# HDembinski/zenflow

Hardware: AMD Instinct MI355X
Metric: log_prob samples/sec (+ NLL match) 4D 16-knot 4-layer flow, batch 2^20 (higher is better)
Workload: dtype fp32 (f16x2 split MFMA, fp32 accumulate)

## Files before the change

include/zenflow_amd.h:

```cpp
#ifndef ZENFLOW_AMD_H
#define ZENFLOW_AMD_H

#include <stddef.h>
#include <stdint.h>

#ifdef __cplusplus
extern "C" {
#endif

#define ZF_OK 0
#define ZF_EINVAL (-1)
#define ZF_ENOTSUP (-2)
#define ZF_ENOMEM (-3)

const char* zf_last_error(void);
int zf_version(void);
int zf_device_count(int* count);
int zf_set_device(int device);
int zf_get_device(int* device);
int zf_device_name(int device, char* buf, int buflen);
int zf_device_synchronize(void);
int zf_malloc(void** ptr, size_t bytes);
int zf_free(void* ptr);
int zf_memset_async(void* ptr, int value, size_t bytes, void* stream);
// ... 69 lines not shown
  int32_t cond_dim;
  int32_t latent;
  float latent_param;
  int32_t n_ops;
  int32_t _pad;
  zf_op_desc ops[64];
} zf_flow_desc;

typedef struct zf_flow zf_flow_t;

int zf_flow_plan(zf_flow_desc* desc, int64_t* blob_floats);

int zf_flow_create(const zf_flow_desc* desc, const float* blob_host, int64_t blob_floats,
                   zf_flow_t** handle);
int zf_flow_destroy(zf_flow_t* handle);

#define ZF_KERNEL_FP32 0
#define ZF_KERNEL_BF16X3 1
#define ZF_KERNEL_F16X2 2
#define ZF_KERNEL_LAYERED 3
int zf_flow_kernel_variant(const zf_flow_t* h);

int64_t zf_flow_workspace_bytes(int64_t N);

int zf_flow_log_prob(zf_flow_t* h, const float* x, const float* c, float* log_prob,
                     double* nll_sum, void* workspace, int64_t N, void* stream);

int zf_flow_log_prob_segment(zf_flow_t* h, int op_begin, int op_end, const float* x,
                             const float* c, const float* log_det_in, float* log_prob,
                             double* nll_sum, void* workspace, int64_t N, void* stream);

int zf_flow_nll_reduce(const void* workspace, int64_t N, double* nll_sum, void* stream);

int zf_flow_forward(zf_flow_t* h, int op_begin, int op_end, const float* x, const float* c,
                    float* y, const float* log_det_in, float* log_det, int64_t N,
                    void* stream);

int zf_flow_inverse(zf_flow_t* h, int op_begin, int op_end, const float* z, const float* c,
                    float* x, int64_t N, void* stream);

int zf_flow_sample(zf_flow_t* h, uint64_t seed, const float* c, float* x, int64_t N, void* stream);

int zf_latent_sample(int latent, double param, uint64_t seed, float* z, int64_t N, int D, void* stream);

int zf_flow_set_bn_stats(zf_flow_t* h, int op, const float* mean, const float* var);

int zf_flow_set_sb_stats(zf_flow_t* h, int op, const float* xmin, const float* xmax);

int64_t zf_colstats_workspace_bytes(int64_t N, int ncols);
int zf_colstats(const float* x, int64_t N, int ncols, int64_t ld, int col_offset,
                const float* pre_modes, const float* pre_params, float* cmin, float* cmax,
                double* csum, double* csumsq, void* workspace, void* stream);


typedef struct zf_optim_desc {
  float learning_rate, b1, b2, eps, weight_decay;
  int nesterov;
} zf_optim_desc;

typedef struct zf_trainer zf_trainer_t;

int zf_trainer_create(const zf_flow_desc* desc, const float* blob_host, int64_t blob_floats,
                      const unsigned char* param_mask, int64_t batch_max, const zf_optim_desc* opt,
                      zf_trainer_t** trainer);
int zf_trainer_destroy(zf_trainer_t* trainer);

// ... 44 lines not shown
```

zenflow_amd/_lib.py:

```python

from __future__ import annotations

import ctypes as C
import os
import threading
import weakref
from pathlib import Path
from typing import Optional, Sequence, Tuple, Union

import numpy as np

_HERE = Path(__file__).resolve().parent
LIB_PATH = Path(os.environ.get("ZF_LIB", _HERE / "libzenflow_amd.so"))

ZF_OP_SHIFT_BOUNDS = 1
ZF_OP_ROLL = 2
ZF_OP_NSC = 3
ZF_LATENT_NONE = 0
ZF_LATENT_NORMAL = 1
ZF_LATENT_BETA = 2
ZF_LATENT_TRUNCNORM = 3
ZF_LATENT_UNIFORM = 4
ZF_ACT_SWISH = 0
ZF_ACT_RELU = 1
ZF_ACT_TANH = 2
ZF_ACT_SIGMOID = 3
ZF_ACT_GELU = 4
ZF_ACT_SOFTPLUS = 5
ZF_ACT_ELU = 6
ZF_ACT_LEAKY_RELU = 7
ZF_SB_NONE = 0
ZF_SB_BOTH = 1
ZF_SB_LOWER = 2
ZF_SB_UPPER = 3
ZF_KERNEL_FP32 = 0
ZF_KERNEL_BF16X3 = 1
ZF_KERNEL_F16X2 = 2
ZF_KERNEL_LAYERED = 3


class ZfOpDesc(C.Structure):
    _fields_ = [
        ("kind", C.c_int32),
        ("shift", C.c_int32),
        ("knots", C.c_int32),
        ("n_hidden", C.c_int32),
        ("hidden", C.c_int32 * 16),
        ("act", C.c_int32),
        ("_pad", C.c_int32),
        ("off_bn", C.c_int64),
        ("off_w", C.c_int64 * 17),
        ("off_b", C.c_int64 * 17),
        ("off_sb", C.c_int64),
    ]


class ZfOptimDesc(C.Structure):
    _fields_ = [("learning_rate", C.c_float), ("b1", C.c_float), ("b2", C.c_float), ("eps", C.c_float),
                ("weight_decay", C.c_float), ("nesterov", C.c_int)]


ALLGATHER_FN = C.CFUNCTYPE(C.c_int, C.c_void_p, C.c_void_p, C.c_void_p, C.c_size_t, C.c_void_p)


class ZfCommDesc(C.Structure):
    _fields_ = [("rank", C.c_int), ("world", C.c_int), ("ctx", C.c_void_p), ("allgather", C.c_void_p)]


class ZfFlowDesc(C.Structure):
    _fields_ = [
        ("dim", C.c_int32),
# ... 18 lines not shown
    "zf_device_count": (_int, [C.POINTER(_int)]),
    "zf_set_device": (_int, [_int]),
    "zf_get_device": (_int, [C.POINTER(_int)]),
    "zf_device_name": (_int, [_int, C.c_char_p, _int]),
    "zf_device_synchronize": (_int, []),
    "zf_malloc": (_int, [C.POINTER(_vp), C.c_size_t]),
    "zf_free": (_int, [_vp]),
    "zf_memset_async": (_int, [_vp, _int, C.c_size_t, _vp]),
    "zf_memcpy_htod": (_int, [_vp, _vp, C.c_size_t, _vp]),
    "zf_memcpy_dtoh": (_int, [_vp, _vp, C.c_size_t, _vp]),
    "zf_memcpy_dtod": (_int, [_vp, _vp, C.c_size_t, _vp]),
    "zf_stream_create": (_int, [C.POINTER(_vp)]),
    "zf_stream_destroy": (_int, [_vp]),
    "zf_stream_synchronize": (_int, [_vp]),
    "zf_event_create": (_int, [C.POINTER(_vp)]),
    "zf_event_destroy": (_int, [_vp]),
    "zf_event_record": (_int, [_vp, _vp]),
    "zf_stream_wait_event": (_int, [_vp, _vp]),
    "zf_event_elapsed_ms": (_int, [_vp, _vp, C.POINTER(C.c_float)]),
    "zf_event_synchronize": (_int, [_vp]),
    "zf_rqs_forward": (_int, [_vp, _vp, _vp, _vp, _vp, _vp, _i64, _int, _int, _vp]),
    "zf_rqs_inverse": (_int, [_vp, _vp, _vp, _vp, _vp, _i64, _int, _int, _vp]),
    "zf_normalize_spline_params": (_int, [_vp, _vp, _vp, _i64, _int, _vp]),
    "zf_squareplus": (_int, [_vp, _vp, _i64, C.c_float, _vp]),
    "zf_softmax_with_threshold": (_int, [_vp, _vp, _i64, _int, C.c_double, _vp]),
    "zf_flow_plan": (_int, [C.POINTER(ZfFlowDesc), C.POINTER(_i64)]),
    "zf_flow_create": (_int, [C.POINTER(ZfFlowDesc), _vp, _i64, C.POINTER(_vp)]),
    "zf_flow_destroy": (_int, [_vp]),
    "zf_flow_kernel_variant": (_int, [_vp]),
    "zf_flow_workspace_bytes": (_i64, [_i64]),
    "zf_flow_log_prob": (_int, [_vp, _vp, _vp, _vp, _vp, _vp, _i64, _vp]),
    "zf_flow_log_prob_segment": (_int, [_vp, _int, _int, _vp, _vp, _vp, _vp, _vp, _vp, _i64, _vp]),
    "zf_flow_nll_reduce": (_int, [_vp, _i64, _vp, _vp]),
    "zf_flow_forward": (_int, [_vp, _int, _int, _vp, _vp, _vp, _vp, _vp, _i64, _vp]),
    "zf_flow_inverse": (_int, [_vp, _int, _int, _vp, _vp, _vp, _i64, _vp]),
    "zf_flow_sample": (_int, [_vp, _u64, _vp, _vp, _i64, _vp]),
    "zf_trainer_create": (_int, [_vp, _vp, _i64, _vp, _i64, _vp, _vp]),
    "zf_trainer_destroy": (_int, [_vp]),
    "zf_trainer_loss_grad": (_int, [_vp, _vp, _vp, _i64, _int, _vp, _vp, _vp]),
    "zf_trainer_step": (_int, [_vp, _vp, _vp, _i64, _vp, _vp]),
    "zf_trainer_set_comm": (_int, [_vp, _vp]),
    "zf_trainer_loss_grad_shard": (_int, [_vp, _vp, _vp, _i64, _i64, _int, _vp, _vp, _vp]),
    "zf_trainer_step_shard": (_int, [_vp, _vp, _vp, _i64, _i64, _vp, _vp]),
    "zf_trainer_loss_grad_cond_shard": (_int, [_vp, _vp, _vp, _i64, _i64, _int, _vp, _vp, _vp, _vp]),
    "zf_trainer_step_cond_shard": (_int, [_vp, _vp, _vp, _i64, _i64, _vp, _vp, _vp]),
    "zf_trainer_log_prob_vjp": (_int, [_vp, _vp, _vp, _vp, _vp, _vp, _vp, _i64, _vp]),
    "zf_trainer_get_blob": (_int, [_vp, _vp]),
    "zf_trainer_set_blob": (_int, [_vp, _vp]),
    "zf_latent_sample": (_int, [_int, _dbl, _u64, _vp, _i64, _int, _vp]),
    "zf_flow_set_bn_stats": (_int, [_vp, _int, _vp, _vp]),
    "zf_flow_set_sb_stats": (_int, [_vp, _int, _vp, _vp]),
    "zf_colstats_workspace_bytes": (_i64, [_i64, _int]),
    "zf_colstats": (_int, [_vp, _i64, _int, _i64, _int, _vp, _vp, _vp, _vp, _vp, _vp, _vp, _vp]),
    "zf_rccl_available": (_int, []),
    "zf_rccl_get_unique_id": (_int, [C.c_char_p]),
    "zf_rccl_comm_init": (_int, [C.POINTER(_vp), _int, C.c_char_p, _int]),
    "zf_rccl_allreduce_sum_f64": (_int, [_vp, _vp, _vp, C.c_size_t, _vp]),
    "zf_rccl_comm_destroy": (_int, [_vp]),
    "zf_rccl_allgather": (_int, [_vp, _vp, _vp, C.c_size_t, _vp]),
}

_lib: Optional[C.CDLL] = None
_lock = threading.Lock()


def load_library() -> C.CDLL:
# ... 207 lines not shown
```

zenflow_amd/csrc/zf_flow.hip:

```cpp
#include "zf_flow_dev.h"

#include <cmath>
#include <cstdlib>
#include <cstring>
#include <vector>

namespace zf {
namespace {

constexpr int kWaves = 4;
constexpr int kBlockRows = kWaves * kTile;

template <int T>
__device__ __forceinline__ floatx16 mfma_tile(const floatx4* __restrict__ p,
                                              const floatx4* __restrict__ pnext, floatx4 (&cur)[4],
                                              const floatx16 (&hb)[T]) {
  floatx16 acc = floatx16{0};
#pragma unroll
  for (int t = 0; t < T; ++t) {
    floatx4 nxt[4];
    const bool more = (t + 1 < T);
    const floatx4* src = more ? p + (t + 1) * 256 : pnext;
    const bool have = more || (pnext != nullptr);
    if (have) {
// ... 288 lines not shown
      if (op.knots < 1 || op.knots > kMaxLayeredKnots)
        return einval("knots %d out of range [1, %d]", op.knots, kMaxLayeredKnots);
      if (op.n_hidden < 1 || op.n_hidden > 16) return enotsup("n_hidden must be in [1, 16]");
      for (int l = 0; l < op.n_hidden; ++l)
        if (op.hidden[l] < 1 || op.hidden[l] > kMaxLayeredWidth)
          return enotsup("hidden width must be in [1, 4096]");
      if (op.act < 0 || op.act >= ZF_ACT_COUNT) return einval("op %d: unknown activation %d", i, op.act);
    } else if (op.kind != ZF_OP_ROLL && op.kind != ZF_OP_SHIFT_BOUNDS) {
      return einval("op %d: unknown kind %d", i, op.kind);
    }
  }
  return ZF_OK;
}

}
}

struct zf_flow {
  zf_flow_desc desc;
  zf::DevFlow host;
  std::vector<float> natural;
  std::vector<float> packed;
  zf::DevFlow* d_desc = nullptr;
  float* d_blob = nullptr;
  void* d_x3 = nullptr;
  int x3_K = 0;
  bool x3_oact = false;
  int x3_aset = 0;
  int device = 0;
  int x3_res_mode = -1;
  int ncu = 0;
  float* d_res_state = nullptr;
  long long res_floats = 0;
  zf::LayeredFlow* lay = nullptr;
};

namespace zf {
namespace {

void pack_nsc_bn(const zf_flow_desc* desc, const zf_op_desc& op, const float* nat, float* dst) {
  const OpGeom g = nsc_geom(desc, op);
  const int DCp = 2 * g.KS0;
  const float* mean = nat + op.off_bn;
  const float* var = mean + g.DC;
  const float* scale = var + g.DC;
  const float* bias = scale + g.DC;
  for (int k = 0; k < DCp; ++k) {
    if (k < g.DC) {
      const float mul = (1.0f / std::sqrt(var[k] + 1e-5f)) * scale[k];
      dst[k] = mean[k];
      dst[DCp + k] = mul;
      dst[2 * DCp + k] = bias[k];
    } else {
      dst[k] = dst[DCp + k] = dst[2 * DCp + k] = 0.f;
    }
  }
}

void pack_sb(const zf_flow_desc* desc, const zf_op_desc& op, const float* nat, float* dst) {
  for (int i = 0; i < desc->dim; ++i) {
    const float* r = nat + op.off_sb + 8 * i;
    const int mode = (int)r[0];
    const float a = r[1], b = r[2], xmin = r[3], xmax = r[4];
    float mul;
    if (mode == ZF_SB_BOTH) mul = (float)(1.0 / ((double)b - (double)a));
    else mul = 1.0f / (xmax - xmin);
// ... 262 lines not shown
}

namespace zf {
namespace {

constexpr int64_t kX3ResidentAutoRows = 1 << 19;

template <bool INV>
int launch_flow(zf_flow* h, int op_begin, int op_end, const float* x, const float* c, float* y,
                const float* ld_in, float* ld_out, float* lp, double* part, int64_t N,
                void* stream, unsigned long long seed = 0, int gen = 0) {
  if (!h) return einval("handle is NULL");
  if (N < 0) return einval("N < 0");
  if (op_begin < 0 || op_end > h->host.n_ops || op_begin > op_end) return einval("bad op range");
  if (N == 0) return ZF_OK;
  if (!x && !gen) return einval("x is NULL");
  if (h->host.C > 0 && !c) return einval("flow is conditional (C=%d) but c is NULL", h->host.C);
  if (h->lay)
    return layered_run(h->lay, h->host, h->d_blob, INV, op_begin, op_end, x, c, y, ld_in, ld_out, lp, part, N,
                       (hipStream_t)stream, seed, gen);
  if (h->host.x3_ok) {
    X3Launch a;
    a.desc = h->d_desc; a.blob = h->d_blob; a.x3 = h->d_x3;
    a.x = x; a.c = c; a.y = y; a.ld_in = ld_in; a.ld_out = ld_out; a.lp = lp; a.part = part;
    a.nparts = (N + kBlockRows - 1) / kBlockRows;
    a.op_begin = op_begin; a.op_end = op_end; a.N = N; a.K = h->x3_K; a.D = h->host.D; a.C = h->host.C; a.T = h->host.HP / 32;
    a.NT = h->host.x3_ok == 2 ? 2 : 3;
    a.oact = h->x3_oact;
    a.aset = h->x3_aset;
    a.par_bytes = h->host.x3_par_bytes;
    a.seed = seed;
    a.gen = gen;
    a.stream = (hipStream_t)stream;
    if (h->x3_res_mode != 0 && (h->x3_res_mode == 1 || N >= kX3ResidentAutoRows) &&
        x3_resident_fits(h->desc, a, INV, h->ncu)) {
      const long long need = ((long long)(N + kTile - 1) / kTile) * kTile * (h->host.D + 1);
      if (need > h->res_floats) {
        hipStreamCaptureStatus cs = hipStreamCaptureStatusNone;
        if (hipStreamIsCapturing(a.stream, &cs) == hipSuccess && cs == hipStreamCaptureStatusNone) {
          if (h->d_res_state) (void)hipFree(h->d_res_state);
          h->d_res_state = nullptr;
          h->res_floats = 0;
          ZF_TRY_HIP(hipMalloc(&h->d_res_state, (size_t)need * sizeof(float)));
          h->res_floats = need;
        }
      }
      if (need <= h->res_floats) a.res_state = h->d_res_state;
    }
    return launch_flow_x3(a, INV);
  }
  const int64_t grid = (N + kBlockRows - 1) / kBlockRows;
  if (grid > 0x7fffffffLL) return einval("N too large");
  const size_t lds = sizeof(float) * (size_t)kWaves * h->host.per_wave;
  if (lds > 160 * 1024 - 64) return enotsup("LDS footprint too large (dim/knots)");
  hipStream_t st = (hipStream_t)stream;
  const long long n = (long long)N;
#define ZF_LAUNCH(HPV)                                                                          \
  hipLaunchKernelGGL((flow_kernel<HPV, INV>), dim3((unsigned)grid), dim3(kWaves * 64), lds, st, \
                     h->d_desc, h->d_blob, x, c, y, ld_in, ld_out, lp, part, op_begin, op_end, n, seed, gen)
  switch (h->host.HP) {
    case 32: ZF_LAUNCH(32); break;
    case 64: ZF_LAUNCH(64); break;
    case 128: ZF_LAUNCH(128); break;
    case 256: ZF_LAUNCH(256); break;
    default: return enotsup("hidden width");
  }
#undef ZF_LAUNCH
  ZF_CHECK_LAUNCH("flow_kernel");
  return ZF_OK;
}

}
}

extern "C" {

int zf_flow_log_prob_segment(zf_flow_t* h, int op_begin, int op_end, const float* x,
                             const float* c, const float* log_det_in, float* log_prob,
                             double* nll_sum, void* workspace, int64_t N, void* stream) {
  if (!h) return zf::einval("handle is NULL");
  if (!log_prob) return zf::einval("log_prob is NULL");
  if (h->host.latent == ZF_LATENT_NONE) return zf::einval("flow has no latent distribution");
  if (nll_sum && !workspace) return zf::einval("nll_sum requires a workspace");
  if (N == 0) {
    if (nll_sum) ZF_TRY_HIP(hipMemsetAsync(nll_sum, 0, sizeof(double), (hipStream_t)stream));
    return ZF_OK;
  }
  double* part = (double*)workspace;
  int rc = zf::launch_flow<false>(h, op_begin, op_end, x, c, nullptr, log_det_in, nullptr,
                                  log_prob, part, N, stream);
  if (rc) return rc;
  if (nll_sum) return zf_flow_nll_reduce(workspace, N, nll_sum, stream);
  return ZF_OK;
}

int zf_flow_nll_reduce(const void* workspace, int64_t N, double* nll_sum, void* stream) {
  if (!workspace || !nll_sum) return zf::einval("NULL argument");
  if (N <= 0) {
    ZF_TRY_HIP(hipMemsetAsync(nll_sum, 0, sizeof(double), (hipStream_t)stream));
    return ZF_OK;
  }
  const long long blocks = (N + zf::kBlockRows - 1) / zf::kBlockRows;
  hipLaunchKernelGGL(zf::reduce_partials, dim3(1), dim3(zf::kReduceThreads), 0, (hipStream_t)stream,
                     (const double*)workspace, blocks, nll_sum);
  ZF_CHECK_LAUNCH("reduce_partials");
  return ZF_OK;
}

int zf_flow_log_prob(zf_flow_t* h, const float* x, const float* c, float* log_prob,
                     double* nll_sum, void* workspace, int64_t N, void* stream) {
  if (!h) return zf::einval("handle is NULL");
  return zf_flow_log_prob_segment(h, 0, h->host.n_ops, x, c, nullptr, log_prob, nll_sum,
                                  workspace, N, stream);
}

int zf_flow_forward(zf_flow_t* h, int op_begin, int op_end, const float* x, const float* c,
                    float* y, const float* log_det_in, float* log_det, int64_t N, void* stream) {
  return zf::launch_flow<false>(h, op_begin, op_end, x, c, y, log_det_in, log_det, nullptr,
                                nullptr, N, stream);
}

int zf_flow_inverse(zf_flow_t* h, int op_begin, int op_end, const float* z, const float* c,
                    float* x, int64_t N, void* stream) {
  if (!x && N > 0) return zf::einval("x is NULL");
  return zf::launch_flow<true>(h, op_begin, op_end, z, c, x, nullptr, nullptr, nullptr, nullptr,
                               N, stream);
}

// ... 56 lines not shown
```

zenflow_amd/csrc/zf_flow_dev.h:

```cpp
#pragma once
#include "zf_act.h"
#include "zf_internal.h"
#include "zf_random.h"
#include "zf_spline.h"

#include <cstdint>
#include <vector>

namespace zf {

typedef float floatx16 __attribute__((ext_vector_type(16)));
typedef float floatx4 __attribute__((ext_vector_type(4)));

constexpr int kTile = 32;
constexpr int kMaxOps = 64;

struct DevOp {
  int kind, shift, K, S;
  int n_hidden, dt, dc, DC;
  int KS0, T_last, nslot_mask, act;
  long long w[17];
  long long b[17];
  long long bn;
  long long sb;
// ... 255 lines not shown
        double acc = 0.0;
        for (int w = 0; w < NW; ++w) acc += s_part[w];
        const long long b0 = slot >= 0 ? slot : (long long)blockIdx.x * pstride;
        block_partial[b0] = acc;
        for (int k = 1; k < pstride; ++k)
          if (b0 + k < nparts) block_partial[b0 + k] = 0.0;
      }
    }
  }
  flow_out_rows(xs, s, hh, rot, D, row, valid, ld, y_out, ld_out);
}

struct X3Launch {
  const DevFlow* desc;
  const float* blob;
  const void* x3;
  const float *x, *c;
  float* y;
  const float* ld_in;
  float *ld_out, *lp;
  double* part;
  long long nparts;
  int op_begin, op_end;
  long long N;
  unsigned long long seed;
  int gen;
  int K, D, C, T;
  int NT;
  bool oact;
  int aset;
  int par_bytes;
  float* res_state = nullptr;
  int res_blocks = 0, res_slots = 0, res_span = 0;
  hipStream_t stream;
};
int launch_flow_x3(const X3Launch& a, bool inverse);
int x3_resident_mode();
bool x3_resident_fits(const zf_flow_desc& desc, X3Launch& a, bool inverse, int ncu);
bool x3_eligible(const zf_flow_desc& desc, int HP, int* K);
struct LayeredFlow;
int layered_create(const zf_flow_desc& desc, const float* natural, int64_t n, LayeredFlow** out);
void layered_destroy(LayeredFlow* L);
int layered_run(LayeredFlow* L, const DevFlow& F, const float* packed, bool inverse, int op_begin, int op_end,
                const float* x, const float* c, float* y, const float* ld_in, float* ld_out, float* lp, double* part,
                long long N, hipStream_t st, unsigned long long seed, int gen);
int x3_last_tiles(int K);
int x3_pairs(const zf_flow_desc& desc);
int x3_buf_tiles(const zf_flow_desc& desc, int T, int K);
size_t x3_lds_bytes(int TB, int D, int NT, int par_bytes);
int x3_scheme();
int x3_scheme_for(const zf_flow_desc& desc);
void x3_pack(const zf_flow_desc& desc, const float* nat, int T, int NT, int Kp, DevFlow& F, float* packed,
             std::vector<uint16_t>& stream);

}
```

zenflow_amd/csrc/zf_flow_x3.hip:

```cpp
#include "zf_flow_x3_kernel.h"

#include <cmath>
#include <cstdint>
#include <cstdlib>
#include <cstring>
#include <vector>

namespace zf {

int launch_x3_k8(const X3Launch& a, bool inverse);
int launch_x3_k16(const X3Launch& a, bool inverse);
int launch_x3_k32(const X3Launch& a, bool inverse);
int launch_x3_k64(const X3Launch& a, bool inverse);

namespace {

uint16_t bf16_rne(float f) {
  uint32_t u;
  std::memcpy(&u, &f, 4);
  if ((u & 0x7fffffffu) > 0x7f800000u) return (uint16_t)((u >> 16) | 0x40);
  u += 0x7fffu + ((u >> 16) & 1u);
  return (uint16_t)(u >> 16);
}

// ... 23 lines not shown
    if (op.act != ZF_ACT_SWISH && x3_scheme() == 3) return false;
    if (op.knots < 2) return false;
    if (op.knots > K) K = op.knots;
  }
  const int Kp = x3_padded_knots(K);
  if (HP > 256 || desc.dim > 64 || Kp == 0) return false;
  *K_out = Kp;
  return true;
}

int x3_resident_mode() {
  const char* env = std::getenv("ZF_X3_RESIDENT");
  if (env && env[0] == '0' && env[1] == 0) return 0;
  if (env && env[0] == '1' && env[1] == 0) return 1;
  return -1;
}

bool x3_resident_fits(const zf_flow_desc& desc, X3Launch& a, bool inverse, int ncu) {
  if (a.NT != 2 || a.T != 4 || a.oact || ncu <= 0 || a.N <= 0) return false;
  const int dt = desc.dim / 2;
  if (dt > 2) return false;
  bool in_range = false;
  for (int i = 0; i < desc.n_ops; ++i) {
    if (desc.ops[i].kind != ZF_OP_NSC) continue;
    if (desc.ops[i].n_hidden != 2) return false;
    if (i >= a.op_begin && i < a.op_end) in_range = true;
  }
  if (!in_range) return false;
  const int TL = dt == 1 ? x3_last_tiles_one(a.K) : x3_last_tiles(a.K);
  const long long span = 4ll * (2 * 4 * 2 * 1024) + 4ll * (2 * TL * 2 * 1024);
  const long long nslots = (a.N + 127) / 128;
  const long long slots = (nslots + ncu - 1) / ncu;
  if (slots > (1 << 20)) return false;
  if (x3_res_lds_bytes((size_t)span, a.par_bytes, a.D + a.C, 4 * slots) > 160 * 1024) return false;
  if (a.K != 16 || dt != 2) return false;
  a.res_blocks = ncu;
  a.res_slots = (int)slots;
  a.res_span = (int)span;
  return true;
}

int x3_padded_knots(int K) {
  if (K < 2) return 0;
  if (K <= 8) return 8;
  if (K <= 16) return 16;
  if (K <= 32) return 32;
  if (K <= 64) return 64;
  return 0;
}

int x3_param_of(int jp, int Kp, int K, float* fill) {
  if (jp < Kp) {
    *fill = -1099511627776.0f;
    return jp < K ? jp : -1;
  }
  if (jp < 2 * Kp) {
    *fill = -1099511627776.0f;
    return jp - Kp < K ? K + (jp - Kp) : -1;
  }
  const int q = jp - 2 * Kp;
  *fill = q == K - 1 ? 0.0f : __builtin_nanf("");
  return q < K - 1 ? 2 * K + q : -1;
}

int x3_scheme() {
  const char* env = std::getenv("ZF_X3_SCHEME");
  if (env && std::strcmp(env, "bf16x3") == 0) return 3;
  return 2;
// ... 198 lines not shown
```

zenflow_amd/csrc/zf_flow_x3_kernel.h:

```cpp
#pragma once
#include "zf_flow_dev.h"

#include <cmath>
#include <cstdint>
#include <cstdlib>
#include <cstring>
#include <utility>
#include <vector>

namespace zf {
namespace {

typedef float floatx2 __attribute__((ext_vector_type(2)));
typedef __bf16 bf16x2 __attribute__((ext_vector_type(2)));
typedef __bf16 bf16x8 __attribute__((ext_vector_type(8)));
typedef _Float16 halfx2 __attribute__((ext_vector_type(2)));
typedef _Float16 halfx8 __attribute__((ext_vector_type(8)));

template <int NT>
struct XT;
template <>
struct XT<3> {
  using E = bf16x8;
  static constexpr int kProd = 6;
// ... 1388 lines not shown
#pragma unroll
        for (int j = 0; j < K - 1; ++j) sl[j] = P[2 * K + j];
#ifndef ZF_X3_EXECBIN
#define ZF_X3_EXECBIN 1
#endif
        const auto spf = [](float v) { return v == 0.f ? 1.f : x3_squareplus_t<OACT>(v); };
        if constexpr (ZF_X3_EXECBIN && K % 8 == 0) bin = rqs_bin_exec<!INV, K>(xv, w, hg, sl, spf, padlast);
        else bin = rqs_bin_monotone<!INV, K>(xv, w, hg, sl, spf, padlast);
        X3M(13);
      }
      float yv;
      if (!INV) {
        float l;
        x3_forward_eval(xv, bin, yv, l);
        ldv = dact ? l : 0.f;
      } else {
        yv = rqs_inverse_eval(xv, bin);
      }
      if (dact) *xp = yv;
    }
    wave_lds_sync();
    if (!INV) {
      const X3Halves q = x3_halves(ldv);
      ldn = ldn + q.lo;
      if (2 * pr + 1 < dt) ldn = ldn + q.hi;
    }
  }
  if (!INV) ld = ld + ldn;
  X3T(5);
}

constexpr int kX3ResWaves = 12;

inline size_t x3_res_lds_bytes(size_t span, int par_bytes, int DS, long long tiles_per_block) {
  return span + (size_t)par_bytes + (size_t)kX3ResWaves * 2 * (DS + 1) * 32 * 4 + (size_t)tiles_per_block * 8;
}

__device__ __forceinline__ void x3r_fetch(const float* __restrict__ st, float* buf, int D, int DS, int lane) {
#pragma nounroll
  for (int j = 0; j < D; j += 2)
    if (j + (lane >> 5) < D)
      __builtin_amdgcn_global_load_lds((const void*)(st + j * 32 + lane),
                                       (__attribute__((address_space(3))) void*)(buf + j * 32), 4, 0, 0);
  if (lane < 32)
    __builtin_amdgcn_global_load_lds((const void*)(st + D * 32 + lane),
                                     (__attribute__((address_space(3))) void*)(buf + DS * 32), 4, 0, 0);
}

template <int K, bool ONE, bool INV>
__global__ __launch_bounds__(kX3ResWaves * 64, 1) void flow_kernel_x3r(
    const DevFlow* __restrict__ F, const float* __restrict__ blob, const char* __restrict__ x3,
    const float* __restrict__ xin, const float* __restrict__ cin, float* __restrict__ y_out,
    const float* __restrict__ ld_in, float* __restrict__ ld_out, float* __restrict__ lp_out,
    double* __restrict__ block_partial, int op_begin, int op_end, long long N, unsigned long long seed, int gen,
    float* __restrict__ state, int slots_per_block, int span_bytes) {
  constexpr int NT = 2, T = 4, NW = kX3ResWaves;
  extern __shared__ __attribute__((aligned(16))) char lds[];
  const int D = F->D;
  const int C = F->C;
  const int wave = __builtin_amdgcn_readfirstlane(threadIdx.x >> 6);
  const int lane = threadIdx.x & 63;
  const int s = lane & 31;
  const int hh = lane >> 5;
  const int PB = F->x3_par_bytes;
  const int DS = D + C;
  const int SB = (DS + 1) * 32;
  const int ST = (D + 1) * 32;
  char* par_lds = lds + span_bytes;
  float* xs0 = reinterpret_cast<float*>(par_lds + PB) + wave * (2 * SB);
  double* s_part = reinterpret_cast<double*>(reinterpret_cast<float*>(par_lds + PB) + NW * 2 * SB);
  const long long slot0 = (long long)blockIdx.x * slots_per_block;
  const long long tile0 = slot0 * 4;
  const long long left = (N + kTile - 1) / kTile - tile0;
  const int nt = left <= 0 ? 0 : (left < 4ll * slots_per_block ? (int)left : 4 * slots_per_block);
  for (int i = threadIdx.x; i < 4 * slots_per_block; i += NW * 64) s_part[i] = 0.0;

  X3Pipe pipe;
  pipe.nxt = nullptr;
  pipe.wave = wave;
  pipe.par_src = nullptr;
  pipe.par_dst = nullptr;
  pipe.par_pieces = 0;
  X3Tr tr = {};
  const int nq = op_end - op_begin;
  int rot0 = 0;
  bool first = true;
  for (int q = 0; q < nq;) {
    int nsc = -1, seg_end = nq;
    for (int r = q; r < nq; ++r)
      if (F->ops[INV ? (op_end - 1 - r) : (op_begin + r)].kind == ZF_OP_NSC) {
        if (nsc < 0) {
          nsc = r;
        } else {
          seg_end = nsc + 1;
          break;
        }
      }
    const bool last = seg_end == nq;
    __syncthreads();
    if (nsc >= 0 && nt > 0) {
      const DevOp& fo = F->ops[INV ? (op_end - 1 - nsc) : (op_begin + nsc)];
      const int pieces = (T * (fo.n_hidden - 1) * group_bytes<NT>(T) + T * group_bytes<NT>(fo.x3_tlast)) >> 10;
      x3_dma(x3 + fo.x3, lds, pieces, wave, lane, NW);
      x3_dma(reinterpret_cast<const char*>(blob + fo.bn), par_lds, fo.x3_par_pieces, wave, lane, NW);
    }
    asm volatile("s_waitcnt vmcnt(0)" ::: "memory");
    __syncthreads();

    int cur = 0;
    if (!first && wave < nt) x3r_fetch(state + (tile0 + wave) * ST, xs0, D, DS, lane);
    for (int t = wave; t < nt; t += NW) {
      float* xs = xs0 + cur * SB;
      const long long tile = tile0 + t;
      int ln = lane;
      asm volatile("" : "+v"(ln));
      {
        const int s1 = ln & 31, h1 = ln >> 5;
        const long long row1 = tile * kTile + s1;
        const bool valid1 = row1 < N;
        if (first) {
          load_state(xs, xin, row1, valid1, D, s1, h1, F, seed, INV ? gen : 0);
        } else if (t == wave) {
          asm volatile("s_waitcnt vmcnt(0)" ::: "memory");
        }
#pragma nounroll
        for (int j = h1; j < C; j += 2) xs[(D + j) * 32 + s1] = valid1 ? cin[row1 * C + j] : 0.f;
      }
      wave_lds_sync();
      float ld;
      if (first) {
        const long long row1 = tile * kTile + (ln & 31);
        ld = (ld_in != nullptr && row1 < N) ? ld_in[row1] : 0.f;
      } else {
        ld = xs[DS * 32 + (ln & 31)];
        if (t + NW < nt) x3r_fetch(state + (tile + NW) * ST, xs0 + (cur ^ 1) * SB, D, DS, ln);
      }
      int rot = rot0;
      for (int r = q; r < seg_end; ++r) {
        const DevOp& op = F->ops[INV ? (op_end - 1 - r) : (op_begin + r)];
        const X3Sc opc = x3_scalars<INV>(op);
        if (opc.kind == ZF_OP_ROLL) {
          rot = pmod(INV ? rot + opc.shift : rot - opc.shift, D);
        } else if (opc.kind == ZF_OP_SHIFT_BOUNDS) {
          shift_bounds_op<INV>(blob + opc.sb, xs, s, hh, rot, D, ld);
        } else {
          int zoff = 0;
          asm volatile("" : "+s"(zoff));
          pipe.cur = lds + zoff;
          pipe.g = 0;
          x3_nsc<NT, K, T, false, ONE, INV, false, 0, true>(
              op, opc, x3, pipe, reinterpret_cast<const float*>(par_lds + zoff), xs, rot, D, s, hh, lane, ld, tr);
        }
      }
      asm volatile("s_waitcnt vmcnt(0)" ::: "memory");
      asm volatile("" : "+v"(ln));
      const int s2 = ln & 31, h2 = ln >> 5;
      const long long row = tile * kTile + s2;
      const bool valid = row < N;
      if (!last) {
        float* st = state + tile * ST;
#pragma nounroll
        for (int d = h2; d < D; d += 2) st[d * 32 + s2] = xs[d * 32 + s2];
        if (h2 == 0) st[D * 32 + s2] = ld;
      } else {
        if (lp_out != nullptr) {
          const double v = flow_lp_rows(F, xs, s2, h2, rot, D, row, valid, ld, lp_out, block_partial != nullptr);
          if (block_partial != nullptr && ln == 0) s_part[t] = v;
        }
        flow_out_rows(xs, s2, h2, rot, D, row, valid, ld, y_out, ld_out);
      }
      wave_lds_sync();
      cur ^= 1;
    }
    for (int r = q; r < seg_end; ++r) {
      const DevOp& op = F->ops[INV ? (op_end - 1 - r) : (op_begin + r)];
      if (op.kind == ZF_OP_ROLL) rot0 = pmod(INV ? rot0 + op.shift : rot0 - op.shift, D);
    }
    q = seg_end;
    first = false;
  }
  __syncthreads();
  if (lp_out != nullptr && block_partial != nullptr) {
    const int ns = (nt + 3) / 4;
    for (int i = threadIdx.x; i < ns; i += NW * 64) {
      double acc = 0.0;
      for (int w = 0; w < 4; ++w) acc += s_part[4 * i + w];
      block_partial[slot0 + i] = acc;
    }
  }
}

template <int K, bool ONE>
int launch_x3r(const X3Launch& a, bool inverse) {
  const size_t lds = x3_res_lds_bytes((size_t)a.res_span, a.par_bytes, a.D + a.C, 4ll * a.res_slots);
  if (lds > 160 * 1024 || a.res_state == nullptr) return enotsup("resident split-MFMA kernel: shape");
  if (inverse)
    hipLaunchKernelGGL((flow_kernel_x3r<K, ONE, true>), dim3((unsigned)a.res_blocks), dim3(kX3ResWaves * 64), lds,
                       a.stream, a.desc, a.blob, (const char*)a.x3, a.x, a.c, a.y, a.ld_in, a.ld_out, a.lp, a.part,
                       a.op_begin, a.op_end, a.N, a.seed, a.gen, a.res_state, a.res_slots, a.res_span);
  else
    hipLaunchKernelGGL((flow_kernel_x3r<K, ONE, false>), dim3((unsigned)a.res_blocks), dim3(kX3ResWaves * 64), lds,
                       a.stream, a.desc, a.blob, (const char*)a.x3, a.x, a.c, a.y, a.ld_in, a.ld_out, a.lp, a.part,
                       a.op_begin, a.op_end, a.N, a.seed, a.gen, a.res_state, a.res_slots, a.res_span);
  ZF_CHECK_LAUNCH("flow_kernel_x3r");
  return ZF_OK;
}

template <int NT, int K, int T, bool PAIRS, bool ONE, bool INV, bool OACT, int ASET = 0>
__global__ __launch_bounds__(kX3Waves * 64, (x3_occupancy<T, K, PAIRS>())) void flow_kernel_x3(
    const DevFlow* __restrict__ F, const float* __restrict__ blob, const char* __restrict__ x3,
    const float* __restrict__ xin, const float* __restrict__ cin, float* __restrict__ y_out,
    const float* __restrict__ ld_in, float* __restrict__ ld_out, float* __restrict__ lp_out,
    double* __restrict__ block_partial, long long nparts, int op_begin, int op_end, long long N,
    unsigned long long seed, int gen) {
  constexpr int TL = ONE ? (3 * K - 1 + 31) / 32 : (3 * K - 1 + 15) / 16;
  constexpr int NW = kX3Waves;
  extern __shared__ __attribute__((aligned(16))) char lds[];
  const int D = F->D;
  const int C = F->C;
  const int wave = __builtin_amdgcn_readfirstlane(threadIdx.x >> 6);
  const int lane = threadIdx.x & 63;
  const int s = lane & 31;
  const int hh = lane >> 5;
  constexpr int kBuf = group_bytes<NT>(T > TL ? T : TL);
  const int PB = F->x3_par_bytes;
  const int DS = D + C;
  char* par_lds = lds + 2 * kBuf;
  float* xs = reinterpret_cast<float*>(par_lds + 2 * PB) + wave * (32 * DS);
  double* s_part = reinterpret_cast<double*>(reinterpret_cast<float*>(par_lds + 2 * PB) + NW * 32 * DS);
  const float* sp = blob;
  const long long row = ((long long)blockIdx.x * NW + wave) * kTile + s;
  const bool valid = row < N;

  X3Pipe pipe;
  pipe.cur = lds;
  pipe.nxt = lds + kBuf;
// ... 130 lines not shown
```

zenflow_amd/engine.py:

```python

from __future__ import annotations

import ctypes as ct
import copy
import math
from dataclasses import dataclass
from typing import Any, Dict, List, Optional, Tuple

import numpy as np

from . import _lib as L
from ._lib import DeviceArray, check
from .module import get_path, set_path

try:
    import xxhash as _xxhash
except ImportError:
    _xxhash = None
import hashlib
from collections import OrderedDict

BN_MOMENTUM = 0.99
BN_EPS = 1e-5

# ... 73 lines not shown
        for i, op in enumerate(self.ops):
            d = desc.ops[i]
            d.kind = op.kind
            if op.kind == L.ZF_OP_ROLL:
                d.shift = int(op.module.shift)
            elif op.kind == L.ZF_OP_NSC:
                m = op.module
                if len(m.layers) < 1:
                    raise NotImplementedError("NeuralSplineCoupling with no hidden layer")
                if len(m.layers) > 16:
                    raise NotImplementedError("more than 16 hidden layers")
                d.knots = int(m.knots)
                d.n_hidden = len(m.layers)
                for l, w in enumerate(m.layers):
                    d.hidden[l] = int(w)
                d.act = int(m.act_code)
        n = ct.c_int64()
        lib = L.load_library()
        check(lib.zf_flow_plan(ct.byref(desc), ct.byref(n)), "zf_flow_plan")
        blob = np.zeros(max(1, n.value), np.float32)
        self.param_mask = np.zeros(blob.shape, np.uint8)
        self._fill_blob(desc, blob, params, stats)
        self.blob = blob
        h = ct.c_void_p()
        check(lib.zf_flow_create(ct.byref(desc), blob.ctypes.data, n.value, ct.byref(h)), "zf_flow_create")
        self.desc = desc
        self.handle = h.value
        self._ws: Optional[DeviceArray] = None

    @property
    def kernel_variant(self) -> str:
        v = L.load_library().zf_flow_kernel_variant(ct.c_void_p(self.handle))
        return {L.ZF_KERNEL_F16X2: "f16x2", L.ZF_KERNEL_BF16X3: "bf16x3", L.ZF_KERNEL_LAYERED: "layered"}.get(v, "fp32")

    def __del__(self):
        h = getattr(self, "handle", None)
        if h and L._lib is not None:
            L._lib.zf_flow_destroy(ct.c_void_p(h))
            self.handle = None

    def _fill_blob(self, desc, blob, params, stats):
        D, Cd = self.D, self.C
        for i, op in enumerate(self.ops):
            d = desc.ops[i]
            if op.kind == L.ZF_OP_SHIFT_BOUNDS:
                st = get_path(stats, op.path) or {}
                for j, (mode, a, b) in enumerate(sb_modes(op.module, D)):
                    xmin = np.asarray(st.get(f"xmin_{j}", [np.inf]), np.float32).reshape(-1)[0]
                    xmax = np.asarray(st.get(f"xmax_{j}", [-np.inf]), np.float32).reshape(-1)[0]
                    blob[d.off_sb + 8 * j : d.off_sb + 8 * j + 6] = [mode, a, b, xmin, xmax, op.module.margin]
            elif op.kind == L.ZF_OP_NSC:
                p = get_path(params, op.path)
                s = get_path(stats, op.path)
                if p is None:
                    raise ValueError(f"missing params for NeuralSplineCoupling at {'/'.join(op.path) or '<root>'}")
                dt = D // 2
                DC = D - dt + Cd
                bnp = p.get("BatchNorm_0", {})
                bns = (s or {}).get("BatchNorm_0", {})
                o = d.off_bn
                blob[o : o + DC] = _arr(bns.get("mean", np.zeros(DC)), (DC,), "BatchNorm_0/mean")
                blob[o + DC : o + 2 * DC] = _arr(bns.get("var", np.ones(DC)), (DC,), "BatchNorm_0/var")
                blob[o + 2 * DC : o + 3 * DC] = _arr(bnp.get("scale", np.ones(DC)), (DC,), "BatchNorm_0/scale")
                blob[o + 3 * DC : o + 4 * DC] = _arr(bnp.get("bias", np.zeros(DC)), (DC,), "BatchNorm_0/bias")
                self.param_mask[o + 2 * DC : o + 4 * DC] = 1
                widths = list(op.module.layers) + [dt * (3 * op.module.knots - 1)]
# ... 248 lines not shown
```

Before: 1.447 billion.

## Add specialized resident kernel frame for 4D unconditional normal-latent flows

```diff
diff --git a/include/zenflow_amd.h b/include/zenflow_amd.h
--- a/include/zenflow_amd.h
+++ b/include/zenflow_amd.h
@@ -125,6 +125,11 @@
 
 int zf_flow_nll_reduce(const void* workspace, int64_t N, double* nll_sum, void* stream);
 
+#define ZF_FORM_STREAMING 0
+#define ZF_FORM_RESIDENT 1
+#define ZF_FORM_RESIDENT_FRAME 2
+int64_t zf_flow_launch_count(const zf_flow_t* h, int form);
+
 int zf_flow_forward(zf_flow_t* h, int op_begin, int op_end, const float* x, const float* c,
                     float* y, const float* log_det_in, float* log_det, int64_t N,
                     void* stream);
diff --git a/zenflow_amd/_lib.py b/zenflow_amd/_lib.py
--- a/zenflow_amd/_lib.py
+++ b/zenflow_amd/_lib.py
@@ -37,6 +37,9 @@
 ZF_KERNEL_BF16X3 = 1
 ZF_KERNEL_F16X2 = 2
 ZF_KERNEL_LAYERED = 3
+ZF_FORM_STREAMING = 0
+ZF_FORM_RESIDENT = 1
+ZF_FORM_RESIDENT_FRAME = 2
 
 
 class ZfOpDesc(C.Structure):
@@ -121,6 +124,7 @@
     "zf_flow_log_prob": (_int, [_vp, _vp, _vp, _vp, _vp, _vp, _i64, _vp]),
     "zf_flow_log_prob_segment": (_int, [_vp, _int, _int, _vp, _vp, _vp, _vp, _vp, _vp, _i64, _vp]),
     "zf_flow_nll_reduce": (_int, [_vp, _i64, _vp, _vp]),
+    "zf_flow_launch_count": (_i64, [_vp, _int]),
     "zf_flow_forward": (_int, [_vp, _int, _int, _vp, _vp, _vp, _vp, _vp, _i64, _vp]),
     "zf_flow_inverse": (_int, [_vp, _int, _int, _vp, _vp, _vp, _i64, _vp]),
     "zf_flow_sample": (_int, [_vp, _u64, _vp, _vp, _i64, _vp]),
diff --git a/zenflow_amd/csrc/zf_flow.hip b/zenflow_amd/csrc/zf_flow.hip
--- a/zenflow_amd/csrc/zf_flow.hip
+++ b/zenflow_amd/csrc/zf_flow.hip
@@ -344,6 +344,7 @@
   int ncu = 0;
   float* d_res_state = nullptr;
   long long res_floats = 0;
+  int64_t n_launch[3] = {0, 0, 0};
   zf::LayeredFlow* lay = nullptr;
 };
 
@@ -672,6 +673,15 @@
     a.seed = seed;
     a.gen = gen;
     a.stream = (hipStream_t)stream;
+    a.latent = h->host.latent;
+    a.sb_affine = true;
+    for (int i = op_begin; i < op_end; ++i) {
+      if (h->desc.ops[i].kind != ZF_OP_SHIFT_BOUNDS) continue;
+      for (int j = 0; j < h->host.D; ++j) {
+        const int mode = (int)h->packed[(size_t)h->host.ops[i].sb + 8 * j];
+        if (mode != ZF_SB_NONE && mode != ZF_SB_BOTH) a.sb_affine = false;
+      }
+    }
     if (h->x3_res_mode != 0 && (h->x3_res_mode == 1 || N >= kX3ResidentAutoRows) &&
         x3_resident_fits(h->desc, a, INV, h->ncu)) {
       const long long need = ((long long)(N + kTile - 1) / kTile) * kTile * (h->host.D + 1);
@@ -687,7 +697,9 @@
       }
       if (need <= h->res_floats) a.res_state = h->d_res_state;
     }
-    return launch_flow_x3(a, INV);
+    const int rc = launch_flow_x3(a, INV);
+    if (rc == ZF_OK) ++h->n_launch[a.res_state == nullptr ? 0 : a.res_frame ? 2 : 1];
+    return rc;
   }
   const int64_t grid = (N + kBlockRows - 1) / kBlockRows;
   if (grid > 0x7fffffffLL) return einval("N too large");
@@ -734,6 +746,11 @@
   return ZF_OK;
 }
 
+int64_t zf_flow_launch_count(const zf_flow_t* h, int form) {
+  if (!h || form < ZF_FORM_STREAMING || form > ZF_FORM_RESIDENT_FRAME) return -1;
+  return h->n_launch[form];
+}
+
 int zf_flow_nll_reduce(const void* workspace, int64_t N, double* nll_sum, void* stream) {
   if (!workspace || !nll_sum) return zf::einval("NULL argument");
   if (N <= 0) {
diff --git a/zenflow_amd/csrc/zf_flow_dev.h b/zenflow_amd/csrc/zf_flow_dev.h
--- a/zenflow_amd/csrc/zf_flow_dev.h
+++ b/zenflow_amd/csrc/zf_flow_dev.h
@@ -311,6 +311,9 @@
   int par_bytes;
   float* res_state = nullptr;
   int res_blocks = 0, res_slots = 0, res_span = 0;
+  bool sb_affine = false;
+  int latent = 0;
+  bool res_frame = false;
   hipStream_t stream;
 };
 int launch_flow_x3(const X3Launch& a, bool inverse);
diff --git a/zenflow_amd/csrc/zf_flow_x3.hip b/zenflow_amd/csrc/zf_flow_x3.hip
--- a/zenflow_amd/csrc/zf_flow_x3.hip
+++ b/zenflow_amd/csrc/zf_flow_x3.hip
@@ -79,8 +79,19 @@
   const long long nslots = (a.N + 127) / 128;
   const long long slots = (nslots + ncu - 1) / ncu;
   if (slots > (1 << 20)) return false;
-  if (x3_res_lds_bytes((size_t)span, a.par_bytes, a.D + a.C, 4 * slots) > 160 * 1024) return false;
+  if (x3_res_lds_bytes((size_t)span, a.par_bytes, a.D + a.C, 4 * slots, false) > 160 * 1024) return false;
   if (a.K != 16 || dt != 2) return false;
+#ifndef ZF_X3R_FRAME
+#define ZF_X3R_FRAME 1
+#endif
+  a.res_frame = ZF_X3R_FRAME && a.D == 4 && a.C == 0 && a.sb_affine && a.latent == ZF_LATENT_NORMAL &&
+                a.ld_in == nullptr;
+  for (int i = a.op_begin, run = 0; i < a.op_end && a.res_frame; ++i) {
+    const int kind = desc.ops[i].kind;
+    run = kind == ZF_OP_NSC ? 0 : run + (kind == ZF_OP_SHIFT_BOUNDS ? 1 : 0);
+    if (run > 1) a.res_frame = false;
+  }
+  if (x3_res_lds_bytes((size_t)span, a.par_bytes, a.D + a.C, 4 * slots, true) > 160 * 1024) a.res_frame = false;
   a.res_blocks = ncu;
   a.res_slots = (int)slots;
   a.res_span = (int)span;
diff --git a/zenflow_amd/csrc/zf_flow_x3_kernel.h b/zenflow_amd/csrc/zf_flow_x3_kernel.h
--- a/zenflow_amd/csrc/zf_flow_x3_kernel.h
+++ b/zenflow_amd/csrc/zf_flow_x3_kernel.h
@@ -1444,8 +1444,9 @@
 
 constexpr int kX3ResWaves = 12;
 
-inline size_t x3_res_lds_bytes(size_t span, int par_bytes, int DS, long long tiles_per_block) {
-  return span + (size_t)par_bytes + (size_t)kX3ResWaves * 2 * (DS + 1) * 32 * 4 + (size_t)tiles_per_block * 8;
+inline size_t x3_res_lds_bytes(size_t span, int par_bytes, int DS, long long tiles_per_block, bool frame) {
+  return span + (size_t)par_bytes + (size_t)kX3ResWaves * 2 * (DS + 1) * 32 * 4 + (size_t)tiles_per_block * 8 +
+         (frame ? 128 : 0);
 }
 
 __device__ __forceinline__ void x3r_fetch(const float* __restrict__ st, float* buf, int D, int DS, int lane) {
@@ -1459,7 +1460,107 @@
                                      (__attribute__((address_space(3))) void*)(buf + DS * 32), 4, 0, 0);
 }
 
-template <int K, bool ONE, bool INV>
+
+struct X3rPass {
+  static __device__ __forceinline__ int pack(int rot_sb_before, int rot_sb_after, int rot_nsc, int rot_end,
+                                             bool sb_before, bool sb_after, int nsc_op) {
+    return rot_sb_before | (rot_sb_after << 2) | (rot_nsc << 4) | (rot_end << 6) | (sb_before ? 1 << 8 : 0) |
+           (sb_after ? 1 << 9 : 0) | (nsc_op << 10);
+  }
+  static __device__ __forceinline__ int rot_sb_before(int p) { return p & 3; }
+  static __device__ __forceinline__ int rot_sb_after(int p) { return (p >> 2) & 3; }
+  static __device__ __forceinline__ int rot_nsc(int p) { return (p >> 4) & 3; }
+  static __device__ __forceinline__ int rot_end(int p) { return (p >> 6) & 3; }
+  static __device__ __forceinline__ bool has_sb_before(int p) { return (p >> 8) & 1; }
+  static __device__ __forceinline__ bool has_sb_after(int p) { return (p >> 9) & 1; }
+  static __device__ __forceinline__ int nsc(int p) { return p >> 10; }
+};
+
+template <bool INV>
+__device__ __forceinline__ floatx4 x3r_sb_consts(const float* __restrict__ sb, int i) {
+  const float* r = sb + 8 * i;
+  const bool both = (int)r[0] == ZF_SB_BOTH;
+  floatx4 k;
+  if (!INV) {
+    float ldsb = 0.f;
+    for (int j = 0; j < 4; ++j) ldsb = ldsb + sb[8 * j + 6];
+    k[0] = both ? r[1] : r[3];
+    k[1] = r[5];
+    k[2] = both ? 0.f : 1.f;
+    k[3] = ldsb;
+  } else {
+    k[0] = both ? r[2] : r[4];
+    k[1] = both ? r[1] : r[3];
+    k[2] = both ? 1.f : 0.f;
+    k[3] = 0.f;
+  }
+  return k;
+}
+
+template <bool INV>
+__device__ __forceinline__ void x3r_shift_bounds(const floatx4* kc, float* xs, int s, int hh, int rot, float& ld) {
+  float ldsb = 0.f;
+#pragma unroll
+  for (int e = 0; e < 2; ++e) {
+    const int i = hh + 2 * e;
+    const floatx4 k = kc[i];
+    float* px = xs + ((i + rot) & 3) * 32 + s;
+    const float v = *px;
+    if (!INV) {
+      const float zr = (v - k[0]) * k[1];
+      *px = (k[2] == 0.f || zr != zr) ? zr : fminf(fmaxf(zr, 0.f), 1.f);
+      ldsb = k[3];
+    } else {
+      const float w = 1.f - v;
+      const float two_sided = __builtin_fmaf(w, k[1], v * k[0]);
+      const float unbounded = __builtin_fmaf(v, k[0], w * k[1]);
+      *px = k[2] != 0.f ? two_sided : unbounded;
+    }
+  }
+  if (!INV) ld = ld + ldsb;
+  wave_lds_sync();
+}
+
+template <int M>
+__device__ __forceinline__ double x3r_from_above(double v) {
+  int lo = __double2loint(v), hi = __double2hiint(v);
+  if constexpr (M == 16) {
+    lo = __builtin_amdgcn_permlane16_swap(lo, lo, false, false)[1];
+    hi = __builtin_amdgcn_permlane16_swap(hi, hi, false, false)[1];
+  } else {
+    constexpr int ctrl = M == 8 ? 0x128 : M == 4 ? 0x104 : M == 2 ? 0x4E : 0xB1;
+    lo = __builtin_amdgcn_update_dpp(lo, lo, ctrl, 0xF, 0xF, false);
+    hi = __builtin_amdgcn_update_dpp(hi, hi, ctrl, 0xF, 0xF, false);
+  }
+  return __hiloint2double(hi, lo);
+}
+
+__device__ __forceinline__ double x3r_lp_rows(float c0, float c1, const float* xs, int s, int hh, int rot, bool valid,
+                                              float ld, float* __restrict__ lp_tile, bool want_sum) {
+  const float ta = latent_logpdf(ZF_LATENT_NORMAL, c0, c1, 0.f, xs[((hh + rot) & 3) * 32 + s]);
+  const float tb = latent_logpdf(ZF_LATENT_NORMAL, c0, c1, 0.f, xs[((hh + 2 + rot) & 3) * 32 + s]);
+  const float oa = x3_halves(ta).hi, ob = x3_halves(tb).hi;
+  float lat = 0.f;
+  lat = lat + ta;
+  lat = lat + oa;
+  lat = lat + tb;
+  lat = lat + ob;
+  const float lp = nan_to_num_lp(lat + ld);
+  if (valid && hh == 0) lp_tile[s] = lp;
+  double v = 0.0;
+  if (want_sum) {
+    v = (valid && hh == 0) ? (double)lp : 0.0;
+    v = v + 0.0;
+    v += x3r_from_above<16>(v);
+    v += x3r_from_above<8>(v);
+    v += x3r_from_above<4>(v);
+    v += x3r_from_above<2>(v);
+    v += x3r_from_above<1>(v);
+  }
+  return v;
+}
+
+template <int K, bool ONE, bool INV, bool FR>
 __global__ __launch_bounds__(kX3ResWaves * 64, 1) void flow_kernel_x3r(
     const DevFlow* __restrict__ F, const float* __restrict__ blob, const char* __restrict__ x3,
     const float* __restrict__ xin, const float* __restrict__ cin, float* __restrict__ y_out,
@@ -1468,8 +1569,8 @@
     float* __restrict__ state, int slots_per_block, int span_bytes) {
   constexpr int NT = 2, T = 4, NW = kX3ResWaves;
   extern __shared__ __attribute__((aligned(16))) char lds[];
-  const int D = F->D;
-  const int C = F->C;
+  const int D = FR ? 4 : F->D;
+  const int C = FR ? 0 : F->C;
   const int wave = __builtin_amdgcn_readfirstlane(threadIdx.x >> 6);
   const int lane = threadIdx.x & 63;
   const int s = lane & 31;
@@ -1497,6 +1598,7 @@
   const int nq = op_end - op_begin;
   int rot0 = 0;
   bool first = true;
+  floatx4* sbk = reinterpret_cast<floatx4*>(s_part + 4 * slots_per_block);
   for (int q = 0; q < nq;) {
     int nsc = -1, seg_end = nq;
     for (int r = q; r < nq; ++r)
@@ -1509,6 +1611,30 @@
         }
       }
     const bool last = seg_end == nq;
+    int fr_pack = 0, fr_sba = -1, fr_sbb = -1;
+    if constexpr (FR) {
+      int fr_nsc = 0, fr_rota = 0, fr_rotb = 0, fr_rotn = 0;
+      int rot = rot0;
+      for (int r = q; r < seg_end; ++r) {
+        const int oi = INV ? (op_end - 1 - r) : (op_begin + r);
+        const int kind = F->ops[oi].kind;
+        if (kind == ZF_OP_ROLL) {
+          rot = (INV ? rot + F->ops[oi].shift : rot - F->ops[oi].shift) & 3;
+        } else if (kind == ZF_OP_SHIFT_BOUNDS) {
+          if (r < nsc) {
+            fr_sba = oi;
+            fr_rota = rot;
+          } else {
+            fr_sbb = oi;
+            fr_rotb = rot;
+          }
+        } else {
+          fr_nsc = oi;
+          fr_rotn = rot;
+        }
+      }
+      fr_pack = X3rPass::pack(fr_rota, fr_rotb, fr_rotn, rot, fr_sba >= 0, fr_sbb >= 0, fr_nsc);
+    }
     __syncthreads();
     if (nsc >= 0 && nt > 0) {
       const DevOp& fo = F->ops[INV ? (op_end - 1 - nsc) : (op_begin + nsc)];
@@ -1516,22 +1642,48 @@
       x3_dma(x3 + fo.x3, lds, pieces, wave, lane, NW);
       x3_dma(reinterpret_cast<const char*>(blob + fo.bn), par_lds, fo.x3_par_pieces, wave, lane, NW);
     }
+    if constexpr (FR) {
+      int lh = lane;
+      asm volatile("" : "+v"(lh));
+      if (wave == 0 && lh < 8) {
+        const int oi = lh < 4 ? fr_sba : fr_sbb;
+        if (oi >= 0) sbk[lh] = x3r_sb_consts<INV>(blob + F->ops[oi].sb, lh & 3);
+      }
+    }
     asm volatile("s_waitcnt vmcnt(0)" ::: "memory");
     __syncthreads();
 
     int cur = 0;
     if (!first && wave < nt) x3r_fetch(state + (tile0 + wave) * ST, xs0, D, DS, lane);
+    float lat_c0 = 0.f, lat_c1 = 1.f;
+    if (FR && last && lp_out != nullptr) {
+      lat_c0 = F->lat_c0;
+      lat_c1 = F->lat_c1;
+    }
     for (int t = wave; t < nt; t += NW) {
       float* xs = xs0 + cur * SB;
       const long long tile = tile0 + t;
+      const long long nleft = N - tile * kTile;
+      const int nrows = nleft < kTile ? (int)nleft : kTile;
       int ln = lane;
       asm volatile("" : "+v"(ln));
       {
         const int s1 = ln & 31, h1 = ln >> 5;
         const long long row1 = tile * kTile + s1;
-        const bool valid1 = row1 < N;
+        const bool valid1 = FR ? s1 < nrows : row1 < N;
         if (first) {
-          load_state(xs, xin, row1, valid1, D, s1, h1, F, seed, INV ? gen : 0);
+          if constexpr (FR) {
+            const float lat_c3 = F->lat_c3;
+            const float* xt = xin + tile * (kTile * 4);
+#pragma unroll
+            for (int d = h1; d < 4; d += 2) {
+              float v = 0.f;
+              if (valid1) v = (INV && gen) ? latent_draw(ZF_LATENT_NORMAL, lat_c3, seed, row1, d) : xt[s1 * 4 + d];
+              xs[d * 32 + s1] = v;
+            }
+          } else {
+            load_state(xs, xin, row1, valid1, D, s1, h1, F, seed, INV ? gen : 0);
+          }
         } else if (t == wave) {
           asm volatile("s_waitcnt vmcnt(0)" ::: "memory");
         }
@@ -1542,38 +1694,75 @@
       float ld;
       if (first) {
         const long long row1 = tile * kTile + (ln & 31);
-        ld = (ld_in != nullptr && row1 < N) ? ld_in[row1] : 0.f;
+        ld = (!FR && ld_in != nullptr && row1 < N) ? ld_in[row1] : 0.f;
       } else {
         ld = xs[DS * 32 + (ln & 31)];
         if (t + NW < nt) x3r_fetch(state + (tile + NW) * ST, xs0 + (cur ^ 1) * SB, D, DS, ln);
       }
       int rot = rot0;
-      for (int r = q; r < seg_end; ++r) {
-        const DevOp& op = F->ops[INV ? (op_end - 1 - r) : (op_begin + r)];
-        const X3Sc opc = x3_scalars<INV>(op);
-        if (opc.kind == ZF_OP_ROLL) {
-          rot = pmod(INV ? rot + opc.shift : rot - opc.shift, D);
-        } else if (opc.kind == ZF_OP_SHIFT_BOUNDS) {
-          shift_bounds_op<INV>(blob + opc.sb, xs, s, hh, rot, D, ld);
-        } else {
+      if constexpr (FR) {
+        int fp = fr_pack;
+        asm volatile("" : "+s"(fp));
+        if (X3rPass::has_sb_before(fp)) x3r_shift_bounds<INV>(sbk, xs, s, hh, X3rPass::rot_sb_before(fp), ld);
+        {
+          const DevOp& op = F->ops[X3rPass::nsc(fp)];
+          const X3Sc opc = x3_scalars<INV>(op);
           int zoff = 0;
           asm volatile("" : "+s"(zoff));
           pipe.cur = lds + zoff;
           pipe.g = 0;
           x3_nsc<NT, K, T, false, ONE, INV, false, 0, true>(
-              op, opc, x3, pipe, reinterpret_cast<const float*>(par_lds + zoff), xs, rot, D, s, hh, lane, ld, tr);
+              op, opc, x3, pipe, reinterpret_cast<const float*>(par_lds + zoff), xs, X3rPass::rot_nsc(fp), 4, s, hh, lane, ld,
+              tr);
+        }
+        asm volatile("" : "+s"(fp));
+        if (X3rPass::has_sb_after(fp)) x3r_shift_bounds<INV>(sbk + 4, xs, s, hh, X3rPass::rot_sb_after(fp), ld);
+        rot = X3rPass::rot_end(fp);
+      } else {
+        for (int r = q; r < seg_end; ++r) {
+          const DevOp& op = F->ops[INV ? (op_end - 1 - r) : (op_begin + r)];
+          const X3Sc opc = x3_scalars<INV>(op);
+          if (opc.kind == ZF_OP_ROLL) {
+            rot = pmod(INV ? rot + opc.shift : rot - opc.shift, D);
+          } else if (opc.kind == ZF_OP_SHIFT_BOUNDS) {
+            shift_bounds_op<INV>(blob + opc.sb, xs, s, hh, rot, D, ld);
+          } else {
+            int zoff = 0;
+            asm volatile("" : "+s"(zoff));
+            pipe.cur = lds + zoff;
+            pipe.g = 0;
+            x3_nsc<NT, K, T, false, ONE, INV, false, 0, true>(
+                op, opc, x3, pipe, reinterpret_cast<const float*>(par_lds + zoff), xs, rot, D, s, hh, lane, ld, tr);
+          }
         }
       }
       asm volatile("s_waitcnt vmcnt(0)" ::: "memory");
       asm volatile("" : "+v"(ln));
       const int s2 = ln & 31, h2 = ln >> 5;
       const long long row = tile * kTile + s2;
-      const bool valid = row < N;
+      const bool valid = FR ? s2 < nrows : row < N;
       if (!last) {
         float* st = state + tile * ST;
+        if constexpr (FR) {
+#pragma unroll
+          for (int d = h2; d < 4; d += 2) st[d * 32 + s2] = xs[d * 32 + s2];
+        } else {
 #pragma nounroll
-        for (int d = h2; d < D; d += 2) st[d * 32 + s2] = xs[d * 32 + s2];
+          for (int d = h2; d < D; d += 2) st[d * 32 + s2] = xs[d * 32 + s2];
+        }
         if (h2 == 0) st[D * 32 + s2] = ld;
+      } else if constexpr (FR) {
+        if (lp_out != nullptr) {
+          const double v = x3r_lp_rows(lat_c0, lat_c1, xs, s2, h2, rot, valid, ld, lp_out + tile * kTile,
+                                       block_partial != nullptr);
+          if (block_partial != nullptr && ln == 0) s_part[t] = v;
+        }
+        if (y_out != nullptr && valid) {
+          float* yt = y_out + tile * (kTile * 4);
+#pragma unroll
+          for (int j = h2; j < 4; j += 2) yt[s2 * 4 + j] = xs[((j + rot) & 3) * 32 + s2];
+        }
+        if (ld_out != nullptr && valid && h2 == 0) (ld_out + tile * kTile)[s2] = ld;
       } else {
         if (lp_out != nullptr) {
           const double v = flow_lp_rows(F, xs, s2, h2, rot, D, row, valid, ld, lp_out, block_partial != nullptr);
@@ -1604,16 +1793,25 @@
 
 template <int K, bool ONE>
 int launch_x3r(const X3Launch& a, bool inverse) {
-  const size_t lds = x3_res_lds_bytes((size_t)a.res_span, a.par_bytes, a.D + a.C, 4ll * a.res_slots);
+  const size_t lds = x3_res_lds_bytes((size_t)a.res_span, a.par_bytes, a.D + a.C, 4ll * a.res_slots, !ONE && a.res_frame);
   if (lds > 160 * 1024 || a.res_state == nullptr) return enotsup("resident split-MFMA kernel: shape");
-  if (inverse)
-    hipLaunchKernelGGL((flow_kernel_x3r<K, ONE, true>), dim3((unsigned)a.res_blocks), dim3(kX3ResWaves * 64), lds,
-                       a.stream, a.desc, a.blob, (const char*)a.x3, a.x, a.c, a.y, a.ld_in, a.ld_out, a.lp, a.part,
-                       a.op_begin, a.op_end, a.N, a.seed, a.gen, a.res_state, a.res_slots, a.res_span);
-  else
-    hipLaunchKernelGGL((flow_kernel_x3r<K, ONE, false>), dim3((unsigned)a.res_blocks), dim3(kX3ResWaves * 64), lds,
-                       a.stream, a.desc, a.blob, (const char*)a.x3, a.x, a.c, a.y, a.ld_in, a.ld_out, a.lp, a.part,
-                       a.op_begin, a.op_end, a.N, a.seed, a.gen, a.res_state, a.res_slots, a.res_span);
+#define ZF_X3R_LAUNCH(INVV, FRV)                                                                                     \
+  hipLaunchKernelGGL((flow_kernel_x3r<K, ONE, INVV, FRV>), dim3((unsigned)a.res_blocks), dim3(kX3ResWaves * 64), lds, \
+                     a.stream, a.desc, a.blob, (const char*)a.x3, a.x, a.c, a.y, a.ld_in, a.ld_out, a.lp, a.part,    \
+                     a.op_begin, a.op_end, a.N, a.seed, a.gen, a.res_state, a.res_slots, a.res_span)
+  if constexpr (!ONE) {
+    if (a.res_frame) {
+      if (inverse) ZF_X3R_LAUNCH(true, true);
+      else ZF_X3R_LAUNCH(false, true);
+    } else {
+      if (inverse) ZF_X3R_LAUNCH(true, false);
+      else ZF_X3R_LAUNCH(false, false);
+    }
+  } else {
+    if (inverse) ZF_X3R_LAUNCH(true, false);
+    else ZF_X3R_LAUNCH(false, false);
+  }
+#undef ZF_X3R_LAUNCH
   ZF_CHECK_LAUNCH("flow_kernel_x3r");
   return ZF_OK;
 }
diff --git a/zenflow_amd/engine.py b/zenflow_amd/engine.py
--- a/zenflow_amd/engine.py
+++ b/zenflow_amd/engine.py
@@ -129,6 +129,11 @@
     def kernel_variant(self) -> str:
         v = L.load_library().zf_flow_kernel_variant(ct.c_void_p(self.handle))
         return {L.ZF_KERNEL_F16X2: "f16x2", L.ZF_KERNEL_BF16X3: "bf16x3", L.ZF_KERNEL_LAYERED: "layered"}.get(v, "fp32")
+
+    def launch_count(self, form: str) -> int:
+        f = {"streaming": L.ZF_FORM_STREAMING, "resident": L.ZF_FORM_RESIDENT,
+             "resident_frame": L.ZF_FORM_RESIDENT_FRAME}[form]
+        return int(L.load_library().zf_flow_launch_count(ct.c_void_p(self.handle), f))
 
     def __del__(self):
         h = getattr(self, "handle", None)
```

New measurement: 1.478 billion (median of 6 runs). 2.1% higher.
